# eridgd/WCT-TF

Measured on AMD Instinct MI355X. Metric: stylized frames/sec @512x512, 5-level relu5->1 pipeline, alpha=0.8, higher is better.
Workload: dtype f16

## Files before the change

### wct_tf_amd/csrc/conv.hip

```cpp
#include "common.h"

typedef unsigned int u32x4 __attribute__((ext_vector_type(4)));
constexpr int TW = 16;
constexpr int PITCH = 20;
constexpr int BK = 32;

__device__ __forceinline__ int reflect_idx(int i, int n) {
  if (i < 0) i = -i;
  if (i >= n) i = 2 * n - 2 - i;
  i = i < 0 ? 0 : i;
  return i >= n ? n - 1 : i;
}

template <int MT, int NT, bool POOL, bool OUT32>
__device__ __forceinline__ void conv_epilogue_t(const ConvArgs& p, f32x16 (&acc)[NT][MT], int b, int y0, int x0, int n0,
                                                int wm, int wn, int lane, const unsigned char* bias_lds) {
  typedef _Float16 h2 __attribute__((ext_vector_type(2)));
  constexpr int OOB = (int)0x80000000u;
  const int frag_px = lane & 15;
  const int frag_py = (lane & 31) >> 4;
  const int kgrp = lane >> 5;
  const int Ho = POOL ? (p.H + 1) / 2 : p.H, Wo = POOL ? (p.W + 1) / 2 : p.W;
  const unsigned img_elems = (unsigned)Ho * Wo * p.Cout;
  const __amdgpu_buffer_rsrc_t r16 = __builtin_amdgcn_make_buffer_rsrc(
// ... 73 lines not shown
        __builtin_amdgcn_raw_buffer_store_b128(o, r16, off16 + (nt * 32 + 16 * m) * 2, 0, 0);
      }
    }
  }
  if (stats) umax_merge(p.umax + b * UMAX_SLOTS, (int)blockIdx.x * 4 + (int)(threadIdx.x >> 6), vmax, lane);
}

template <int MT, int NT>
__device__ __forceinline__ void conv_epilogue(const ConvArgs& p, f32x16 (&acc)[NT][MT], int b, int y0, int x0, int n0,
                                              int wm, int wn, int lane, const unsigned char* bias_lds) {
  if (p.pool) conv_epilogue_t<MT, NT, true, false>(p, acc, b, y0, x0, n0, wm, wn, lane, bias_lds);
  else if (p.y32) conv_epilogue_t<MT, NT, false, true>(p, acc, b, y0, x0, n0, wm, wn, lane, bias_lds);
  else conv_epilogue_t<MT, NT, false, false>(p, acc, b, y0, x0, n0, wm, wn, lane, bias_lds);
}

template <int TH, int BN, int WM, int WN, bool FUSE1 = false>
__global__ __launch_bounds__(256, ((TH / 2) / WM) * ((BN / 32) / WN) > 8 ? 1 : 2) void conv3x3_mfma_kernel(ConvArgs p, int tiles_x, int tiles_y, int n_tiles, int strip) {
  constexpr int PH = TH + 2;
  constexpr int MT = (TH / 2) / WM;
  constexpr int NT = (BN / 32) / WN;
  constexpr int PATCH_ITEMS = PH * 18 * 4;
  constexpr int PATCH_PER_THREAD = (PATCH_ITEMS + 255) / 256;
  constexpr int PATCH_BYTES = PH * PITCH * 64;
  constexpr bool DB = MT * NT > 8;
  constexpr int NBUF = DB ? 2 : 1;
  constexpr int DUMP_OFF = PATCH_BYTES;
  constexpr int BUF_STRIDE = PATCH_BYTES + 4096;
  constexpr int BIAS_OFF = NBUF * BUF_STRIDE;
  constexpr int IMG_OFF = BIAS_OFF + BN * 4, IMG_H = TH + 4, IMG_W = 20, IMG_ROW = IMG_W * 3, IMG_ZERO = IMG_OFF + IMG_H * IMG_ROW * 4;
  constexpr int W1_OFF = IMG_ZERO + 64, B1_OFF = W1_OFF + 8192;
  constexpr int STG_OFF = B1_OFF + 256;
  static_assert(!FUSE1 || (BN == 64 && !(((TH / 2) / WM) * ((BN / 32) / WN) > 8)), "FUSE1: 64 output channels, single patch buffer");
  constexpr int PF_TAP = TH <= 16 ? 6 : 9;

  extern __shared__ __attribute__((aligned(16))) unsigned char smem[];
  unsigned char* const patch_lds = smem;

  int bid = blockIdx.x;
  const int ntile = bid % n_tiles;
  bid /= n_tiles;
  const int strips_x = FUSE1 ? (tiles_x + strip - 1) / strip : tiles_x;
  const int tx = FUSE1 ? (bid % strips_x) * strip : bid % strips_x;
  const int ty = bid / strips_x;
  const int b = blockIdx.y;
  int y0 = ty * TH;
  int x0 = tx * TW;
  int strip_i = 0;
  const int n0 = ntile * BN;
  int tid_ = threadIdx.x;

next_tile:
  if (FUSE1) asm volatile("" : "+v"(tid_), "+s"(y0));
  const int tid = tid_;
  const int lane = tid & 63;
  const int wave = tid >> 6;
  const int wm = wave / WN, wn = wave % WN;

  const int Hin = p.upsample ? p.H / 2 : p.H;
  const int Win = p.upsample ? p.W / 2 : p.W;
  const half_t* xb = p.x + (size_t)b * Hin * Win * p.Cin;

  unsigned patch_src[PATCH_PER_THREAD];
  unsigned patch_dst[PATCH_PER_THREAD];
#pragma unroll
  for (int i = 0; i < PATCH_PER_THREAD; ++i) {
    int item = tid + i * 256;
    int valid = item < PATCH_ITEMS;
    int pix = valid ? item >> 2 : 0;
    int chunk = item & 3;
    int py = pix / 18, px = pix - py * 18;
    int iy = reflect_idx(y0 - 1 + py, p.H);
    int ix = reflect_idx(x0 - 1 + px, p.W);
    if (p.upsample) { iy >>= 1; ix >>= 1; }
    patch_src[i] = valid ? ((iy * Win + ix) * p.Cin + chunk * 8) * 2 : 0;
    patch_dst[i] = valid ? ((py * PITCH + px) * 4 + (chunk ^ ((px >> 2) & 3))) * 16 : DUMP_OFF + tid * 16;
  }

  const int frag_px = lane & 15;
  const int frag_py = (lane & 31) >> 4;
  const int kgrp = lane >> 5;

  int rd_base[3][2];
#pragma unroll
  for (int kx = 0; kx < 3; ++kx)
#pragma unroll
    for (int ks = 0; ks < 2; ++ks) {
      const int px = frag_px + kx;
      rd_base[kx][ks] = ((wm * MT * 2 + frag_py) * PITCH + px) * 64 + (((ks * 2 + kgrp) ^ ((px >> 2) & 3)) * 16);
    }

  const int c16 = p.Cin >> 4;
  unsigned wfrag[NT];
#pragma unroll
  for (int nt = 0; nt < NT; ++nt)
    wfrag[nt] = (((n0 >> 5) + wn * NT + nt) * 9 * c16 * 512 + lane * 8) * 2;
  const __amdgpu_buffer_rsrc_t w_rsrc = __builtin_amdgcn_make_buffer_rsrc((void*)p.w, 0, 0x7FFFFFFF, 0x00020000);
  const __amdgpu_buffer_rsrc_t x_rsrc = __builtin_amdgcn_make_buffer_rsrc((void*)xb, 0, 0x7FFFFFFF, 0x00020000);

  f32x16 acc[NT][MT];
  if (tid < BN / 4 && strip_i == 0)
    *reinterpret_cast<f32x4*>(smem + BIAS_OFF + tid * 16) = *reinterpret_cast<const f32x4*>(p.bias + n0 + tid * 4);

  const int n_chunks = p.Cin / BK;
  u32x4 patch_regs[PATCH_PER_THREAD];
  half8 wf[2][NT][2];
  half8 bf[2][MT];

  auto read_group = [&](half8 (&dst)[MT], int ky, int kx, int ks, int buf) {
#pragma unroll
    for (int mt = 0; mt < MT; ++mt)
      dst[mt] = *reinterpret_cast<const half8*>(patch_lds + rd_base[kx][ks] + (mt * 2 + ky) * PITCH * 64 + buf * BUF_STRIDE);
  };
  auto mma_group = [&](half8 (&w)[NT][2], half8 (&bq)[MT], int ks) {
#pragma unroll
    for (int mt = 0; mt < MT; ++mt)
#pragma unroll
      for (int nt = 0; nt < NT; ++nt)
        acc[nt][mt] = __builtin_amdgcn_mfma_f32_32x32x16_f16(w[nt][ks], bq[mt], acc[nt][mt], 0, 0, 0);
  };
  auto load_patch = [&](int chunk) {
#pragma unroll
    for (int i = 0; i < PATCH_PER_THREAD; ++i)
      patch_regs[i] = __builtin_amdgcn_raw_buffer_load_b128(x_rsrc, patch_src[i], chunk * BK * 2, 0);
  };
  auto store_patch = [&](int buf) {
#pragma unroll
// ... 123 lines not shown
  } else {
    load_patch(0);
  }
#pragma unroll
  for (int nt = 0; nt < NT; ++nt)
#pragma unroll
    for (int ks = 0; ks < 2; ++ks)
      wf[0][nt][ks] = __builtin_bit_cast(half8, __builtin_amdgcn_raw_buffer_load_b128(w_rsrc, wfrag[nt] + ks * 1024, 0, 0));
  if (FUSE1) {
    __syncthreads();
    make_patch(0);
  } else {
    store_patch(0);
  }
  __syncthreads();
  read_group(bf[0], 0, 0, 0, 0);

#pragma unroll 1
  for (int pair = 0; pair < n_chunks; pair += 2) {
#pragma unroll
    for (int t = 0; t < 18; ++t) {
      const int tap = t % 9, chunk_i = pair + t / 9;
      const int ky = tap / 3, kx = tap % 3;
      const int ntap = (tap + 1) % 9, nky = ntap / 3, nkx = ntap % 3;
      const bool more = chunk_i + 1 < n_chunks;
      const int buf = DB ? t / 9 : 0;
      {
        const int nchunk = tap == 8 ? (more ? chunk_i + 1 : chunk_i) : chunk_i;
        const int wtap = (ntap * c16 + nchunk * 2) * 1024;
#pragma unroll
        for (int nt = 0; nt < NT; ++nt)
#pragma unroll
          for (int ks = 0; ks < 2; ++ks)
            wf[(t + 1) & 1][nt][ks] =
                __builtin_bit_cast(half8, __builtin_amdgcn_raw_buffer_load_b128(w_rsrc, wfrag[nt] + ks * 1024, wtap, 0));
      }
      if (!FUSE1 && tap == PF_TAP && more) load_patch(chunk_i + 1);
      read_group(bf[1], ky, kx, 1, buf);
      if (DB && tap == 8 && more) store_patch(buf ^ 1);
      __builtin_amdgcn_sched_barrier(0);
      mma_group(wf[t & 1], bf[0], 0);
      __builtin_amdgcn_sched_barrier(0);
      if (tap != 8) {
        read_group(bf[0], nky, nkx, 0, buf);
        __builtin_amdgcn_sched_barrier(0);
        mma_group(wf[t & 1], bf[1], 1);
      } else {
        mma_group(wf[t & 1], bf[1], 1);
        if (more) {
          __syncthreads();
          if (FUSE1) {
            make_patch(chunk_i + 1);
            __syncthreads();
          } else if (!DB) {
            if (PF_TAP > 8) load_patch(chunk_i + 1);
            store_patch(0);
            __syncthreads();
          }
        }
        read_group(bf[0], 0, 0, 0, DB ? buf ^ 1 : 0);
      }
      __builtin_amdgcn_sched_barrier(0);
    }
  }
  const bool more_tiles = FUSE1 && strip_i + 1 < strip && tx + strip_i + 1 < tiles_x;
  if (more_tiles) fetch_img(x0 + TW);
  conv_epilogue<MT, NT>(p, acc, b, y0, x0, n0, wm, wn, lane, smem + BIAS_OFF);
  if (more_tiles) {
    ++strip_i;
    x0 += TW;
    goto next_tile;
  }
}

template <int TH, int BN, int WM, int WN, bool FUSE1 = false>
static int launch_conv_cfg(const ConvArgs& a, hipStream_t s) {
  const int tiles_x = cdiv(a.W, TW), tiles_y = cdiv(a.H, TH);
  const int n_tiles = a.Cout / BN;
  constexpr int PH = TH + 2;
  constexpr int NBUF = ((TH / 2) / WM) * ((BN / 32) / WN) > 8 ? 2 : 1;
  const size_t lds = (size_t)NBUF * (PH * PITCH * 64 + 4096) + BN * sizeof(float)
                     + (FUSE1 ? (size_t)(TH + 4) * 20 * 3 * 4 + 64 + 8192 + 256 + 9 * 1024 : 0);
  const long tiles = (long)tiles_x * tiles_y * a.B;
  const int strip = !FUSE1 ? 1 : tiles >= 8192 ? 4 : tiles >= 4096 ? 2 : 1;
  dim3 grid((FUSE1 ? cdiv(tiles_x, strip) : tiles_x) * tiles_y * n_tiles, a.B);
  if (lds > 64 * 1024) {
    static bool raised[16] = {};
    int dev = 0;
    HIP_TRY(hipGetDevice(&dev));
    if (dev >= 0 && dev < 16 && !raised[dev]) {
      HIP_TRY(hipFuncSetAttribute(reinterpret_cast<const void*>(&conv3x3_mfma_kernel<TH, BN, WM, WN, FUSE1>),
                                  hipFuncAttributeMaxDynamicSharedMemorySize, (int)lds));
      raised[dev] = true;
    }
  }
  hipLaunchKernelGGL((conv3x3_mfma_kernel<TH, BN, WM, WN, FUSE1>), grid, dim3(256), lds, s, a, tiles_x, tiles_y, n_tiles, strip);
  HIP_TRY(hipGetLastError());
  return WCT_OK;
}

int launch_conv3x3(const ConvArgs& a, hipStream_t s) {
  ARG_CHECK(a.Cin % 64 == 0 && a.Cout % 64 == 0 && a.H > 1 && a.W > 1 && a.B > 0);
  ARG_CHECK(!a.upsample || (a.H % 2 == 0 && a.W % 2 == 0));
  ARG_CHECK((size_t)a.H * a.W * a.Cin * 2 < ((size_t)1 << 31));
  ARG_CHECK((size_t)a.H * a.W * a.Cout * (a.y32 ? 4 : 2) < ((size_t)1 << 31));
  ARG_CHECK(!a.usum || (a.y32 && a.umax && a.relu && a.W % 16 == 0));
  ARG_CHECK(!a.pool || (a.relu && !a.y32));
  if (conv3x3_wino_takes(a)) return launch_conv3x3_wino(a, s);
  if (a.img1) {
    ARG_CHECK(a.Cin == 64 && a.Cout == 64 && !a.upsample && a.w1frag && a.bias1);
    return launch_conv_cfg<32, 64, 4, 1, true>(a, s);
  }
  const long px16 = (long)cdiv(a.W, TW) * cdiv(a.H, 16) * a.B;
  const long px32 = (long)cdiv(a.W, TW) * cdiv(a.H, 32) * a.B;
  if (a.Cout % 128 == 0 && px16 * (a.Cout / 128) >= 512) return launch_conv_cfg<16, 128, 2, 2>(a, s);
  if (px32 * (a.Cout / 64) >= 512) return launch_conv_cfg<32, 64, 4, 1>(a, s);
  if (a.Cout % 128 == 0 && px16 * (a.Cout / 128) >= 256) return launch_conv_cfg<16, 128, 2, 2>(a, s);
  if (px16 * (a.Cout / 64) >= 256) return launch_conv_cfg<16, 64, 4, 1>(a, s);
  return launch_conv_cfg<8, 64, 2, 2>(a, s);
}

__global__ __launch_bounds__(256) void conv_first_kernel(ConvFirstArgs p, int strips_x) {
  constexpr int CF_TILES = 4, PATCH_N = 18 * 18 * 3, PER = (PATCH_N + 255) / 256;
  __shared__ float patch[PATCH_N + 4];
  __shared__ __attribute__((aligned(16))) unsigned char tr[4][32 * 256];
  typedef unsigned int u32x4 __attribute__((ext_vector_type(4)));
  const int tid = threadIdx.x, lane = tid & 63, wave = tid >> 6;
  const int sx = blockIdx.x % strips_x, ty = blockIdx.x / strips_x;
  const int b = blockIdx.y;
  const int y0 = ty * 16;
  const float* xb = p.x + (size_t)b * p.H * p.W * 3;
  int e_row[PER], e_px[PER], e_c[PER];
#pragma unroll
  for (int i = 0; i < PER; ++i) {
// ... 286 lines not shown
```

### wct_tf_amd/csrc/conv_wino.hip

```cpp
#include "common.h"

namespace {
typedef unsigned int u32x4 __attribute__((ext_vector_type(4)));
typedef _Float16 h2 __attribute__((ext_vector_type(2)));
constexpr int TW = 16;
constexpr int PITCH = 20;
constexpr int BK = 32;

__device__ __forceinline__ half8 pk_sub(half8 a, half8 b) {
  u32x4 ua = __builtin_bit_cast(u32x4, a), ub = __builtin_bit_cast(u32x4, b), r;
#pragma unroll
  for (int i = 0; i < 4; ++i) {
    unsigned o;
    asm("v_pk_add_f16 %0, %1, %2 neg_lo:[0,1] neg_hi:[0,1]" : "=v"(o) : "v"(ua[i]), "v"(ub[i]));
    r[i] = o;
  }
  return __builtin_bit_cast(half8, r);
}

__device__ __forceinline__ int reflect_idx(int i, int n) {
  if (i < 0) i = -i;
  if (i >= n) i = 2 * n - 2 - i;
  i = i < 0 ? 0 : i;
  return i >= n ? n - 1 : i;
}

template <int TH, int BN, int WM, int WN, bool IL>
__global__ __launch_bounds__(256, TH >= 16 ? 1 : 2)
void conv3x3_wino_kernel(ConvArgs p, int tiles_x, int n_tiles) {
  constexpr int PR = TH / 2;
  constexpr int MT = (PR / 2) / WM;
  constexpr int NT = (BN / 32) / WN;
  constexpr int G = 256 / PR;
  constexpr int SL = (72 + G - 1) / G;
  constexpr int PATCH_BYTES = PR * 4 * PITCH * 64;
  constexpr int DUMP_OFF = 2 * PATCH_BYTES;
  constexpr int PF_TAP = 5;
  static_assert(PR % 2 == 0 && (PR / 2) % WM == 0 && 256 % PR == 0 && WM * WN == 4, "tile shape");

  extern __shared__ __attribute__((aligned(16))) unsigned char smem[];
  const int tid = threadIdx.x, lane = tid & 63, wave = tid >> 6;
  const int wm = wave / WN, wn = wave % WN;
  int bid = blockIdx.x;
  const int ntile = bid % n_tiles;
  bid /= n_tiles;
  const int tx = bid % tiles_x, ty = bid / tiles_x;
  const int b = blockIdx.y;
  const int y0 = ty * TH, x0 = tx * TW, n0 = ntile * BN;

  const int Hin = p.upsample ? p.H / 2 : p.H;
  const int Win = p.upsample ? p.W / 2 : p.W;
  const half_t* xb = p.x + (size_t)b * Hin * Win * p.Cin;
  const __amdgpu_buffer_rsrc_t w_rsrc = __builtin_amdgcn_make_buffer_rsrc((void*)p.w_wino, 0, 0x7FFFFFFF, 0x00020000);
  const __amdgpu_buffer_rsrc_t x_rsrc = __builtin_amdgcn_make_buffer_rsrc((void*)xb, 0, 0x7FFFFFFF, 0x00020000);

  const int lpr = tid / G, ls = tid % G;
  unsigned row_off[4], col_off[SL], dst_off[SL];
  bool slot_ok[SL];
#pragma unroll
  for (int i = 0; i < 4; ++i) {
    int iy = reflect_idx(y0 + 2 * lpr - 1 + i, p.H);
    if (p.upsample) iy >>= 1;
    row_off[i] = (unsigned)(iy * Win) * p.Cin * 2;
  }
#pragma unroll
  for (int j = 0; j < SL; ++j) {
    const int slot = ls + j * G;
    slot_ok[j] = slot < 72;
    const int px = slot_ok[j] ? slot >> 2 : 0, piece = slot & 3;
    int ix = reflect_idx(x0 - 1 + px, p.W);
    if (p.upsample) ix >>= 1;
    col_off[j] = (unsigned)(ix * p.Cin + piece * 8) * 2;
    dst_off[j] = ((lpr * 4 * PITCH + px) * 4 + (piece ^ ((px >> 2) & 3))) * 16;
    if (IL && !slot_ok[j]) dst_off[j] = DUMP_OFF + tid * 16;
  }
  u32x4 raw[SL][4];
  auto load_rows = [&](int chunk) {
#pragma unroll
    for (int j = 0; j < SL; ++j)
#pragma unroll
      for (int i = 0; i < 4; ++i)
        raw[j][i] = __builtin_amdgcn_raw_buffer_load_b128(x_rsrc, row_off[i] + col_off[j], chunk * BK * 2, 0);
  };
  auto park_rows = [&](int buf) {
#pragma unroll
    for (int j = 0; j < SL; ++j) {
      const half8 d0 = __builtin_bit_cast(half8, raw[j][0]), d1 = __builtin_bit_cast(half8, raw[j][1]);
      const half8 d2 = __builtin_bit_cast(half8, raw[j][2]), d3 = __builtin_bit_cast(half8, raw[j][3]);
      const half8 t0 = pk_sub(d0, d2), t1 = d1 + d2, t2 = pk_sub(d2, d1), t3 = pk_sub(d1, d3);
      if (slot_ok[j]) {
        unsigned char* d = smem + buf * PATCH_BYTES + dst_off[j];
        *reinterpret_cast<half8*>(d) = t0;
        *reinterpret_cast<half8*>(d + PITCH * 64) = t1;
        *reinterpret_cast<half8*>(d + 2 * PITCH * 64) = t2;
        *reinterpret_cast<half8*>(d + 3 * PITCH * 64) = t3;
      }
    }
  };

  const int frag_px = lane & 15, frag_pr = (lane & 31) >> 4, kgrp = lane >> 5;
  int rd_base[3][2];
#pragma unroll
  for (int kx = 0; kx < 3; ++kx)
#pragma unroll
    for (int ks = 0; ks < 2; ++ks) {
      const int px = frag_px + kx;
      rd_base[kx][ks] = (((wm * MT * 2 + frag_pr) * 4) * PITCH + px) * 64 + (((ks * 2 + kgrp) ^ ((px >> 2) & 3)) * 16);
    }
  const int c16 = p.Cin >> 4;
  unsigned wfrag[NT];
#pragma unroll
  for (int nt = 0; nt < NT; ++nt) wfrag[nt] = (((n0 >> 5) + wn * NT + nt) * 12 * c16 * 512 + lane * 8) * 2;

  f32x16 acc[4][NT][MT];
#pragma unroll
  for (int nt = 0; nt < NT; ++nt) {
    f32x4 bv[4];
#pragma unroll
    for (int rq = 0; rq < 4; ++rq) bv[rq] = *reinterpret_cast<const f32x4*>(p.bias + n0 + (wn * NT + nt) * 32 + 8 * rq + 4 * kgrp);
#pragma unroll
    for (int f = 0; f < 4; ++f)
#pragma unroll
      for (int mt = 0; mt < MT; ++mt)
#pragma unroll
        for (int r = 0; r < 16; ++r) acc[f][nt][mt][r] = f == 1 ? bv[r >> 2][r & 3] : 0.f;
  }

  const int n_chunks = p.Cin / BK;
  half8 wf[3][NT][2];
  half8 bf[IL ? 3 : 2][2][MT];
  auto load_w = [&](half8 (&dst)[NT][2], int tap12, int chunk) {
    const int soff = (tap12 * c16 + chunk * 2) * 1024;
#pragma unroll
    for (int nt = 0; nt < NT; ++nt)
#pragma unroll
      for (int ks = 0; ks < 2; ++ks)
// ... 2 lines not shown
  auto read_b = [&](half8 (&dst)[2][MT], int f, int kx, int buf) {
#pragma unroll
    for (int ks = 0; ks < 2; ++ks)
#pragma unroll
      for (int mt = 0; mt < MT; ++mt)
        dst[ks][mt] = *reinterpret_cast<const half8*>(smem + buf * PATCH_BYTES + rd_base[kx][ks] + (mt * 8 + f) * PITCH * 64);
  };

  if constexpr (IL) {
    constexpr int NM = 2 * MT * NT;
    constexpr int NR = 2 * NT + 2 * MT;
#ifndef WINO_LT0
#define WINO_LT0 1
#define WINO_PT0 6
#endif
    constexpr int LT0 = WINO_LT0, PT0 = WINO_PT0;
    static_assert(LT0 + SL <= PT0 && PT0 + SL <= 10, "staging schedule");
#ifndef WINO_WRING
#define WINO_WRING 4
#endif
#ifndef WINO_ABL
#define WINO_ABL 0
#endif
#ifndef WINO_RAW_AUX
#define WINO_RAW_AUX 0
#endif
    constexpr int ABL = WINO_ABL;
    constexpr int WR = WINO_WRING, WA = WR - 1;
    static_assert(24 % WR == 0, "ring");
    half8 wq[WR][NT][2];
    half8 tq[4];
    load_rows(0);
#pragma unroll
    for (int i = 0; i < WA; ++i) load_w(wq[i], i, 0);
#pragma unroll
    for (int j = 0; j < SL; ++j) {
      const half8 d0 = __builtin_bit_cast(half8, raw[j][0]), d1 = __builtin_bit_cast(half8, raw[j][1]);
      const half8 d2 = __builtin_bit_cast(half8, raw[j][2]), d3 = __builtin_bit_cast(half8, raw[j][3]);
      unsigned char* d = smem + dst_off[j];
      *reinterpret_cast<half8*>(d) = pk_sub(d0, d2);
      *reinterpret_cast<half8*>(d + PITCH * 64) = d1 + d2;
      *reinterpret_cast<half8*>(d + 2 * PITCH * 64) = pk_sub(d2, d1);
      *reinterpret_cast<half8*>(d + 3 * PITCH * 64) = pk_sub(d1, d3);
    }
    asm volatile("s_waitcnt lgkmcnt(0)\n\ts_barrier" ::: "memory");
    read_b(bf[0], 0, 0, 0);
    read_b(bf[1], 0, 1, 0);
#pragma unroll 1
    for (int pair = 0; pair < n_chunks; pair += 2) {
#pragma unroll
      for (int t = 0; t < 24; ++t) {
        const int tt = t % 12, chunk_i = pair + t / 12, buf = t / 12;
        const int f = tt / 3, kx = tt % 3;
        const int chunk_n = chunk_i + 1 < n_chunks ? chunk_i + 1 : chunk_i;
        const int t3 = (tt + WA) % 12, c3 = tt + WA >= 12 ? chunk_n : chunk_i;
        const int t1 = (tt + 2) % 12, buf1 = tt >= 10 ? buf ^ 1 : buf;
        const int soff3 = (t3 * c16 + c3 * 2) * 1024;
#pragma unroll
        for (int j = 0; j < NM; ++j) {
          const int ks = j / (MT * NT), mt = (j / NT) % MT, nt = j % NT;
          if (!(ABL & 4)) acc[f][nt][mt] = __builtin_amdgcn_mfma_f32_32x32x16_f16(wq[t % WR][nt][ks], bf[t % 3][ks][mt], acc[f][nt][mt], 0, 0, 0);
          else asm volatile("" :: "v"(wq[t % WR][nt][ks]), "v"(bf[t % 3][ks][mt]));
#pragma unroll
          for (int k = j * NR / NM; k < (j + 1) * NR / NM; ++k) {
            if (k < 2 * NT) {
              if (!(ABL & 1)) wq[(t + WA) % WR][k / 2][k % 2] =
                  __builtin_bit_cast(half8, __builtin_amdgcn_raw_buffer_load_b128(w_rsrc, wfrag[k / 2] + (k % 2) * 1024, soff3, 0));
            } else {
              const int kk = k - 2 * NT, ks1 = kk / MT, mt1 = kk % MT;
              if (!(ABL & 8)) bf[(t + 2) % 3][ks1][mt1] = *reinterpret_cast<const half8*>(smem + buf1 * PATCH_BYTES + rd_base[t1 % 3][ks1] + (mt1 * 8 + t1 / 3) * PITCH * 64);
            }
          }
          if (tt >= LT0 && tt < LT0 + SL) {
            const int sl = tt - LT0;
            if (j < 4 && !(ABL & 2)) raw[sl][j] = __builtin_amdgcn_raw_buffer_load_b128(x_rsrc, (ABL & 64) ? (lane & 3) * 16 + j * 64 + sl * 256 : row_off[j] + col_off[sl], (ABL & 32) ? 0 : chunk_n * BK * 2, WINO_RAW_AUX);
          }
          if (tt >= PT0 && tt < PT0 + SL && !(ABL & 16)) {
            const int sl = tt - PT0;
            {
#pragma unroll
              for (int it = j * 8 / NM; it < (j + 1) * 8 / NM; ++it) {
                const int fq = it >> 1;
                if ((it & 1) == 0) {
                  const half8 da = __builtin_bit_cast(half8, raw[sl][fq == 0 ? 0 : fq == 1 ? 1 : fq == 2 ? 2 : 1]);
                  const half8 db = __builtin_bit_cast(half8, raw[sl][fq == 0 ? 2 : fq == 1 ? 2 : fq == 2 ? 1 : 3]);
                  tq[fq] = fq == 1 ? da + db : pk_sub(da, db);
                } else {
                  *reinterpret_cast<half8*>(smem + (buf ^ 1) * PATCH_BYTES * (slot_ok[sl] ? 1 : 0) + dst_off[sl] + fq * PITCH * 64) = tq[fq];
                }
              }
            }
          }
          __builtin_amdgcn_sched_barrier(0);
        }
        if (tt == 9) asm volatile("s_waitcnt lgkmcnt(0)\n\ts_barrier" ::: "memory");
      }
    }
  } else {
  load_rows(0);
  load_w(wf[0], 0, 0);
  load_w(wf[1], 1, 0);
  park_rows(0);
  asm volatile("s_waitcnt lgkmcnt(0)\n\ts_barrier" ::: "memory");
  read_b(bf[0], 0, 0, 0);

#pragma unroll 1
  for (int pair = 0; pair < n_chunks; pair += 2) {
#pragma unroll
    for (int t = 0; t < 24; ++t) {
      const int tt = t % 12, chunk_i = pair + t / 12, buf = t / 12;
      const int f = tt / 3, kx = tt % 3;
      const bool more = chunk_i + 1 < n_chunks;
      {
        const int t2 = (tt + 2) % 12;
        const int c2 = tt + 2 >= 12 ? (more ? chunk_i + 1 : chunk_i) : chunk_i;
        load_w(wf[(t + 2) % 3], t2, c2);
      }
      if (tt == PF_TAP && more) load_rows(chunk_i + 1);
      if (tt != 11) read_b(bf[(t + 1) & 1], (tt + 1) / 3, (tt + 1) % 3, buf);
      else if (more) read_b(bf[(t + 1) & 1], 0, 0, buf ^ 1);
      __builtin_amdgcn_sched_barrier(0);
#pragma unroll
      for (int ks = 0; ks < 2; ++ks)
#pragma unroll
        for (int mt = 0; mt < MT; ++mt)
#pragma unroll
          for (int nt = 0; nt < NT; ++nt)
            acc[f][nt][mt] = __builtin_amdgcn_mfma_f32_32x32x16_f16(wf[t % 3][nt][ks], bf[t & 1][ks][mt], acc[f][nt][mt], 0, 0, 0);
      __builtin_amdgcn_sched_barrier(0);
      if (tt == 10 && more) {
        park_rows(buf ^ 1);
        asm volatile("s_waitcnt lgkmcnt(0)\n\ts_barrier" ::: "memory");
      }
    }
  }

  }
  constexpr int OOB = (int)0x80000000u;
  const int Ho = p.pool ? (p.H + 1) / 2 : p.H, Wo = p.pool ? (p.W + 1) / 2 : p.W;
  const unsigned img_elems = (unsigned)Ho * Wo * p.Cout;
  const __amdgpu_buffer_rsrc_t r16 = __builtin_amdgcn_make_buffer_rsrc((void*)(p.y16 + (size_t)b * img_elems), 0, img_elems * 2, 0x00020000);
  const float lo1 = p.relu ? 0.f : -__builtin_inff();
  const h2 lo2 = {(half_t)lo1, (half_t)lo1};
  const h2 zero2 = {(half_t)0.f, (half_t)0.f};
  const int ox = x0 + frag_px;
// ... 7 lines not shown
      off[0] = in0 && (frag_px & 1) == 0 ? (((oy >> 1) * Wo + (ox >> 1)) * p.Cout + chan + 8 * kgrp) * 2 : OOB;
      off[1] = OOB;
    } else {
      off[0] = in0 ? ((oy * p.W + ox) * p.Cout + chan + 8 * kgrp) * 2 : OOB;
      off[1] = in1 ? (((oy + 1) * p.W + ox) * p.Cout + chan + 8 * kgrp) * 2 : OOB;
    }
#pragma unroll
    for (int nt = 0; nt < NT; ++nt) {
      unsigned pk[2][4][2];
#pragma unroll
      for (int rq = 0; rq < 4; ++rq) {
        f32x4 e, o;
#pragma unroll
        for (int j = 0; j < 4; ++j) {
          const int r = rq * 4 + j;
          const float m0 = acc[0][nt][mt][r], m1 = acc[1][nt][mt][r], m2 = acc[2][nt][mt][r], m3 = acc[3][nt][mt][r];
          e[j] = (m0 + m1) + m2;
          o[j] = (m1 - m2) - m3;
        }
        h2 e0 = {(half_t)e[0], (half_t)e[1]}, e1 = {(half_t)e[2], (half_t)e[3]};
        h2 o0 = {(half_t)o[0], (half_t)o[1]}, o1 = {(half_t)o[2], (half_t)o[3]};
        e0 = __builtin_elementwise_max(e0, lo2); e1 = __builtin_elementwise_max(e1, lo2);
        o0 = __builtin_elementwise_max(o0, lo2); o1 = __builtin_elementwise_max(o1, lo2);
        if (p.pool) {
          h2 q[2] = {__builtin_elementwise_max(in0 ? e0 : zero2, in1 ? o0 : zero2), __builtin_elementwise_max(in0 ? e1 : zero2, in1 ? o1 : zero2)};
#pragma unroll
          for (int d = 0; d < 2; ++d) {
            const unsigned tq = __builtin_bit_cast(unsigned, q[d]);
            const h2 nb = __builtin_bit_cast(h2, __builtin_amdgcn_update_dpp(0, (int)tq, 0xB1, 0xF, 0xF, true));
            q[d] = __builtin_elementwise_max(q[d], nb);
          }
          e0 = q[0]; e1 = q[1];
        }
// ... 2 lines not shown
      }
#pragma unroll
      for (int par = 0; par < 2; ++par) {
#pragma unroll
        for (int m = 0; m < 2; ++m) {
          auto sx = __builtin_amdgcn_permlane32_swap(pk[par][2 * m][0], pk[par][2 * m + 1][0], false, false);
          auto sy = __builtin_amdgcn_permlane32_swap(pk[par][2 * m][1], pk[par][2 * m + 1][1], false, false);
          u32x4 ov = {sx[0], sy[0], sx[1], sy[1]};
          __builtin_amdgcn_raw_buffer_store_b128(ov, r16, off[par] + (nt * 32 + 16 * m) * 2, 0, 0);
        }
      }
    }
  }
}

template <int TH, int BN, int WM, int WN, bool IL = false>
int launch_wino_cfg(const ConvArgs& a, hipStream_t s) {
  const int tiles_x = cdiv(a.W, TW), tiles_y = cdiv(a.H, TH), n_tiles = a.Cout / BN;
  const size_t lds = 2 * (size_t)(TH / 2) * 4 * PITCH * 64 + (IL ? 8192 : 0);
  HIP_TRY(hipFuncSetAttribute(reinterpret_cast<const void*>(&conv3x3_wino_kernel<TH, BN, WM, WN, IL>),
                              hipFuncAttributeMaxDynamicSharedMemorySize, (int)lds));
  hipLaunchKernelGGL((conv3x3_wino_kernel<TH, BN, WM, WN, IL>), dim3(tiles_x * tiles_y * n_tiles, a.B), dim3(256), lds, s, a, tiles_x, n_tiles);
  HIP_TRY(hipGetLastError());
  return WCT_OK;
}
}

bool conv3x3_wino_takes(const ConvArgs& a) {
  return a.w_wino != nullptr && a.y16 != nullptr && a.y32 == nullptr && a.usum == nullptr && a.img1 == nullptr &&
         a.Cin % 64 == 0 && a.Cout % 64 == 0 && (!a.pool || a.relu);
}

int launch_conv3x3_wino(const ConvArgs& a, hipStream_t s) {
  ARG_CHECK(conv3x3_wino_takes(a) && a.H > 1 && a.W > 1 && a.B > 0);
  ARG_CHECK(!a.upsample || (a.H % 2 == 0 && a.W % 2 == 0));
  ARG_CHECK((size_t)a.H * a.W * a.Cin * 2 < ((size_t)1 << 31));
  ARG_CHECK((size_t)a.H * a.W * a.Cout * 2 < ((size_t)1 << 31));
  const long px16 = (long)cdiv(a.W, TW) * cdiv(a.H, 16) * a.B;
  const long px8 = (long)cdiv(a.W, TW) * cdiv(a.H, 8) * a.B;
  if (a.Cout % 128 == 0 && px16 * (a.Cout / 128) >= 256) return launch_wino_cfg<16, 128, 1, 4, true>(a, s);
  if (a.Cout % 128 == 0 && px8 * (a.Cout / 128) >= 256) return launch_wino_cfg<8, 128, 1, 4>(a, s);
  return launch_wino_cfg<8, 64, 2, 2>(a, s);
}
```

Baseline: 662.6.

## Specialize 3x3 convs with fused nearest upsample to exploit duplicated input rows

Adds an UP template path to both the direct MFMA conv and the Winograd conv, used when the conv input is a 2x nearest-upsampled activation. The direct kernel stages only the half-resolution patch with 8 channel chunks per pixel and reads it with remapped, swizzled LDS addressing. It also refreshes the patch only every other chunk, which cuts global loads and barriers. The Winograd kernel uses the fact that adjacent upsampled rows are equal: it drops one of the four row-transform planes (3 filters and 9 taps instead of 4 and 12) and shortens the MFMA loop and the epilogue. The cost is more complex indexing, extra template instantiations and a larger register and LDS footprint, with correctness depending on the reflection and duplication mapping being right at tile edges.

```diff
diff --git a/wct_tf_amd/csrc/conv.hip b/wct_tf_amd/csrc/conv.hip
--- a/wct_tf_amd/csrc/conv.hip
+++ b/wct_tf_amd/csrc/conv.hip
@@ -111,14 +111,18 @@
   else conv_epilogue_t<MT, NT, false, false>(p, acc, b, y0, x0, n0, wm, wn, lane, bias_lds);
 }
 
-template <int TH, int BN, int WM, int WN, bool FUSE1 = false>
+template <int TH, int BN, int WM, int WN, bool FUSE1 = false, bool UP = false>
 __global__ __launch_bounds__(256, ((TH / 2) / WM) * ((BN / 32) / WN) > 8 ? 1 : 2) void conv3x3_mfma_kernel(ConvArgs p, int tiles_x, int tiles_y, int n_tiles, int strip) {
-  constexpr int PH = TH + 2;
+  constexpr int PH = UP ? TH / 2 + 2 : TH + 2;
   constexpr int MT = (TH / 2) / WM;
   constexpr int NT = (BN / 32) / WN;
-  constexpr int PATCH_ITEMS = PH * 18 * 4;
+  constexpr int PW = UP ? 10 : 18;
+  constexpr int PP = UP ? 11 : PITCH;
+  constexpr int PC = UP ? 8 : 4;
+  constexpr int PXB = PC * 16;
+  constexpr int PATCH_ITEMS = PH * PW * PC;
   constexpr int PATCH_PER_THREAD = (PATCH_ITEMS + 255) / 256;
-  constexpr int PATCH_BYTES = PH * PITCH * 64;
+  constexpr int PATCH_BYTES = PH * PP * PXB;
   constexpr bool DB = MT * NT > 8;
   constexpr int NBUF = DB ? 2 : 1;
   constexpr int DUMP_OFF = PATCH_BYTES;
@@ -127,6 +131,7 @@
   constexpr int IMG_OFF = BIAS_OFF + BN * 4, IMG_H = TH + 4, IMG_W = 20, IMG_ROW = IMG_W * 3, IMG_ZERO = IMG_OFF + IMG_H * IMG_ROW * 4;
   constexpr int W1_OFF = IMG_ZERO + 64, B1_OFF = W1_OFF + 8192;
   constexpr int STG_OFF = B1_OFF + 256;
+  static_assert(!UP || (!FUSE1 && !DB), "UP: activations in, single patch buffer");
   static_assert(!FUSE1 || (BN == 64 && !(((TH / 2) / WM) * ((BN / 32) / WN) > 8)), "FUSE1: 64 output channels, single patch buffer");
   constexpr int PF_TAP = TH <= 16 ? 6 : 9;
 
@@ -153,8 +158,8 @@
   const int wave = tid >> 6;
   const int wm = wave / WN, wn = wave % WN;
 
-  const int Hin = p.upsample ? p.H / 2 : p.H;
-  const int Win = p.upsample ? p.W / 2 : p.W;
+  const int Hin = UP ? p.H / 2 : p.H;
+  const int Win = UP ? p.W / 2 : p.W;
   const half_t* xb = p.x + (size_t)b * Hin * Win * p.Cin;
 
   unsigned patch_src[PATCH_PER_THREAD];
@@ -163,14 +168,15 @@
   for (int i = 0; i < PATCH_PER_THREAD; ++i) {
     int item = tid + i * 256;
     int valid = item < PATCH_ITEMS;
-    int pix = valid ? item >> 2 : 0;
-    int chunk = item & 3;
-    int py = pix / 18, px = pix - py * 18;
-    int iy = reflect_idx(y0 - 1 + py, p.H);
-    int ix = reflect_idx(x0 - 1 + px, p.W);
-    if (p.upsample) { iy >>= 1; ix >>= 1; }
+    int pix = valid ? item / PC : 0;
+    int chunk = item % PC;
+    int py = pix / PW, px = pix - py * PW;
+    int iy = reflect_idx(UP ? (py == 0 ? y0 - 1 : y0 + 2 * (py - 1)) : y0 - 1 + py, p.H);
+    int ix = reflect_idx(UP ? (px == 0 ? x0 - 1 : x0 + 2 * (px - 1)) : x0 - 1 + px, p.W);
+    if (UP) { iy >>= 1; ix >>= 1; }
+    const int sw = UP ? (px >> 1) ^ ((px & 1) << 2) : (px >> 2) & 3;
     patch_src[i] = valid ? ((iy * Win + ix) * p.Cin + chunk * 8) * 2 : 0;
-    patch_dst[i] = valid ? ((py * PITCH + px) * 4 + (chunk ^ ((px >> 2) & 3))) * 16 : DUMP_OFF + tid * 16;
+    patch_dst[i] = valid ? ((py * PP + px) * PC + (chunk ^ sw)) * 16 : DUMP_OFF + tid * 16;
   }
 
   const int frag_px = lane & 15;
@@ -182,8 +188,13 @@
   for (int kx = 0; kx < 3; ++kx)
 #pragma unroll
     for (int ks = 0; ks < 2; ++ks) {
-      const int px = frag_px + kx;
-      rd_base[kx][ks] = ((wm * MT * 2 + frag_py) * PITCH + px) * 64 + (((ks * 2 + kgrp) ^ ((px >> 2) & 3)) * 16);
+      if (UP) {
+        const int c = (frag_px + kx + 1) >> 1, row = wm * MT + (ks ? 1 : frag_py);
+        rd_base[kx][ks] = (row * PP + c) * PXB + ((((c >> 1) ^ ((c & 1) << 2)) ^ kgrp) * 16);
+      } else {
+        const int px = frag_px + kx;
+        rd_base[kx][ks] = ((wm * MT * 2 + frag_py) * PITCH + px) * 64 + (((ks * 2 + kgrp) ^ ((px >> 2) & 3)) * 16);
+      }
     }
 
   const int c16 = p.Cin >> 4;
@@ -203,10 +214,17 @@
   half8 wf[2][NT][2];
   half8 bf[2][MT];
 
-  auto read_group = [&](half8 (&dst)[MT], int ky, int kx, int ks, int buf) {
-#pragma unroll
-    for (int mt = 0; mt < MT; ++mt)
-      dst[mt] = *reinterpret_cast<const half8*>(patch_lds + rd_base[kx][ks] + (mt * 2 + ky) * PITCH * 64 + buf * BUF_STRIDE);
+  auto read_group = [&](half8 (&dst)[MT], int ky, int kx, int ks, int buf, int hf) {
+    if (UP) {
+      const int a = rd_base[kx][ky == 1] ^ ((hf * 4 + ks * 2) * 16);
+#pragma unroll
+      for (int mt = 0; mt < MT; ++mt)
+        dst[mt] = *reinterpret_cast<const half8*>(patch_lds + a + (mt + (ky == 2)) * PP * PXB);
+    } else {
+#pragma unroll
+      for (int mt = 0; mt < MT; ++mt)
+        dst[mt] = *reinterpret_cast<const half8*>(patch_lds + rd_base[kx][ks] + (mt * 2 + ky) * PITCH * 64 + buf * BUF_STRIDE);
+    }
   };
   auto mma_group = [&](half8 (&w)[NT][2], half8 (&bq)[MT], int ks) {
 #pragma unroll
@@ -360,10 +378,14 @@
     store_patch(0);
   }
   __syncthreads();
-  read_group(bf[0], 0, 0, 0, 0);
+  read_group(bf[0], 0, 0, 0, 0, 0);
 
 #pragma unroll 1
   for (int pair = 0; pair < n_chunks; pair += 2) {
+    if (UP) {
+#pragma unroll
+      for (int i = 0; i < 6; ++i) asm volatile("" : "+v"(rd_base[i / 2][i % 2]));
+    }
 #pragma unroll
     for (int t = 0; t < 18; ++t) {
       const int tap = t % 9, chunk_i = pair + t / 9;
@@ -371,6 +393,7 @@
       const int ntap = (tap + 1) % 9, nky = ntap / 3, nkx = ntap % 3;
       const bool more = chunk_i + 1 < n_chunks;
       const int buf = DB ? t / 9 : 0;
+      const int hf = UP ? t / 9 : 0;
       {
         const int nchunk = tap == 8 ? (more ? chunk_i + 1 : chunk_i) : chunk_i;
         const int wtap = (ntap * c16 + nchunk * 2) * 1024;
@@ -381,19 +404,19 @@
             wf[(t + 1) & 1][nt][ks] =
                 __builtin_bit_cast(half8, __builtin_amdgcn_raw_buffer_load_b128(w_rsrc, wfrag[nt] + ks * 1024, wtap, 0));
       }
-      if (!FUSE1 && tap == PF_TAP && more) load_patch(chunk_i + 1);
-      read_group(bf[1], ky, kx, 1, buf);
+      if (!FUSE1 && tap == PF_TAP && more && (!UP || hf)) load_patch(chunk_i + 1);
+      read_group(bf[1], ky, kx, 1, buf, hf);
       if (DB && tap == 8 && more) store_patch(buf ^ 1);
       __builtin_amdgcn_sched_barrier(0);
       mma_group(wf[t & 1], bf[0], 0);
       __builtin_amdgcn_sched_barrier(0);
       if (tap != 8) {
-        read_group(bf[0], nky, nkx, 0, buf);
+        read_group(bf[0], nky, nkx, 0, buf, hf);
         __builtin_amdgcn_sched_barrier(0);
         mma_group(wf[t & 1], bf[1], 1);
       } else {
         mma_group(wf[t & 1], bf[1], 1);
-        if (more) {
+        if (more && (!UP || hf)) {
           __syncthreads();
           if (FUSE1) {
             make_patch(chunk_i + 1);
@@ -404,7 +427,7 @@
             __syncthreads();
           }
         }
-        read_group(bf[0], 0, 0, 0, DB ? buf ^ 1 : 0);
+        read_group(bf[0], 0, 0, 0, DB ? buf ^ 1 : 0, hf ^ (UP ? 1 : 0));
       }
       __builtin_amdgcn_sched_barrier(0);
     }
@@ -419,13 +442,13 @@
   }
 }
 
-template <int TH, int BN, int WM, int WN, bool FUSE1 = false>
+template <int TH, int BN, int WM, int WN, bool FUSE1 = false, bool UP = false>
 static int launch_conv_cfg(const ConvArgs& a, hipStream_t s) {
   const int tiles_x = cdiv(a.W, TW), tiles_y = cdiv(a.H, TH);
   const int n_tiles = a.Cout / BN;
-  constexpr int PH = TH + 2;
+  constexpr int PH = UP ? TH / 2 + 2 : TH + 2;
   constexpr int NBUF = ((TH / 2) / WM) * ((BN / 32) / WN) > 8 ? 2 : 1;
-  const size_t lds = (size_t)NBUF * (PH * PITCH * 64 + 4096) + BN * sizeof(float)
+  const size_t lds = (size_t)NBUF * ((UP ? PH * 11 * 128 : PH * PITCH * 64) + 4096) + BN * sizeof(float)
                      + (FUSE1 ? (size_t)(TH + 4) * 20 * 3 * 4 + 64 + 8192 + 256 + 9 * 1024 : 0);
   const long tiles = (long)tiles_x * tiles_y * a.B;
   const int strip = !FUSE1 ? 1 : tiles >= 8192 ? 4 : tiles >= 4096 ? 2 : 1;
@@ -435,12 +458,12 @@
     int dev = 0;
     HIP_TRY(hipGetDevice(&dev));
     if (dev >= 0 && dev < 16 && !raised[dev]) {
-      HIP_TRY(hipFuncSetAttribute(reinterpret_cast<const void*>(&conv3x3_mfma_kernel<TH, BN, WM, WN, FUSE1>),
+      HIP_TRY(hipFuncSetAttribute(reinterpret_cast<const void*>(&conv3x3_mfma_kernel<TH, BN, WM, WN, FUSE1, UP>),
                                   hipFuncAttributeMaxDynamicSharedMemorySize, (int)lds));
       raised[dev] = true;
     }
   }
-  hipLaunchKernelGGL((conv3x3_mfma_kernel<TH, BN, WM, WN, FUSE1>), grid, dim3(256), lds, s, a, tiles_x, tiles_y, n_tiles, strip);
+  hipLaunchKernelGGL((conv3x3_mfma_kernel<TH, BN, WM, WN, FUSE1, UP>), grid, dim3(256), lds, s, a, tiles_x, tiles_y, n_tiles, strip);
   HIP_TRY(hipGetLastError());
   return WCT_OK;
 }
@@ -459,11 +482,13 @@
   }
   const long px16 = (long)cdiv(a.W, TW) * cdiv(a.H, 16) * a.B;
   const long px32 = (long)cdiv(a.W, TW) * cdiv(a.H, 32) * a.B;
-  if (a.Cout % 128 == 0 && px16 * (a.Cout / 128) >= 512) return launch_conv_cfg<16, 128, 2, 2>(a, s);
-  if (px32 * (a.Cout / 64) >= 512) return launch_conv_cfg<32, 64, 4, 1>(a, s);
-  if (a.Cout % 128 == 0 && px16 * (a.Cout / 128) >= 256) return launch_conv_cfg<16, 128, 2, 2>(a, s);
-  if (px16 * (a.Cout / 64) >= 256) return launch_conv_cfg<16, 64, 4, 1>(a, s);
-  return launch_conv_cfg<8, 64, 2, 2>(a, s);
+#define CONV_CFG(...) (a.upsample ? launch_conv_cfg<__VA_ARGS__, false, true>(a, s) : launch_conv_cfg<__VA_ARGS__>(a, s))
+  if (a.Cout % 128 == 0 && px16 * (a.Cout / 128) >= 512) return CONV_CFG(16, 128, 2, 2);
+  if (px32 * (a.Cout / 64) >= 512) return CONV_CFG(32, 64, 4, 1);
+  if (a.Cout % 128 == 0 && px16 * (a.Cout / 128) >= 256) return CONV_CFG(16, 128, 2, 2);
+  if (px16 * (a.Cout / 64) >= 256) return CONV_CFG(16, 64, 4, 1);
+  return CONV_CFG(8, 64, 2, 2);
+#undef CONV_CFG
 }
 
 __global__ __launch_bounds__(256) void conv_first_kernel(ConvFirstArgs p, int strips_x) {
diff --git a/wct_tf_amd/csrc/conv_wino.hip b/wct_tf_amd/csrc/conv_wino.hip
--- a/wct_tf_amd/csrc/conv_wino.hip
+++ b/wct_tf_amd/csrc/conv_wino.hip
@@ -25,17 +25,23 @@
   return i >= n ? n - 1 : i;
 }
 
-template <int TH, int BN, int WM, int WN, bool IL>
+template <int TH, int BN, int WM, int WN, bool IL, bool UP>
 __global__ __launch_bounds__(256, TH >= 16 ? 1 : 2)
 void conv3x3_wino_kernel(ConvArgs p, int tiles_x, int n_tiles) {
   constexpr int PR = TH / 2;
   constexpr int MT = (PR / 2) / WM;
   constexpr int NT = (BN / 32) / WN;
   constexpr int G = 256 / PR;
-  constexpr int SL = (72 + G - 1) / G;
+  constexpr int NF = UP ? 3 : 4;
+  constexpr int NTAP = NF * 3;
+  constexpr int NRAW = UP ? 3 : 4;
+  constexpr int NS = UP ? 40 : 72;
+  constexpr int SL = (NS + G - 1) / G;
   constexpr int PATCH_BYTES = PR * 4 * PITCH * 64;
   constexpr int DUMP_OFF = 2 * PATCH_BYTES;
-  constexpr int PF_TAP = 5;
+  constexpr int PF_TAP = NTAP - 7;
+  auto FQ = [](int i) { return UP && i == 2 ? 3 : i; };
+  auto TAP12 = [](int t) { return UP && t >= 6 ? t + 3 : t; };
   static_assert(PR % 2 == 0 && (PR / 2) % WM == 0 && 256 % PR == 0 && WM * WN == 4, "tile shape");
 
   extern __shared__ __attribute__((aligned(16))) unsigned char smem[];
@@ -48,43 +54,68 @@
   const int b = blockIdx.y;
   const int y0 = ty * TH, x0 = tx * TW, n0 = ntile * BN;
 
-  const int Hin = p.upsample ? p.H / 2 : p.H;
-  const int Win = p.upsample ? p.W / 2 : p.W;
+  const bool ups = UP || p.upsample;
+  const int Hin = ups ? p.H / 2 : p.H;
+  const int Win = ups ? p.W / 2 : p.W;
   const half_t* xb = p.x + (size_t)b * Hin * Win * p.Cin;
   const __amdgpu_buffer_rsrc_t w_rsrc = __builtin_amdgcn_make_buffer_rsrc((void*)p.w_wino, 0, 0x7FFFFFFF, 0x00020000);
   const __amdgpu_buffer_rsrc_t x_rsrc = __builtin_amdgcn_make_buffer_rsrc((void*)xb, 0, 0x7FFFFFFF, 0x00020000);
 
   const int lpr = tid / G, ls = tid % G;
-  unsigned row_off[4], col_off[SL], dst_off[SL];
-  bool slot_ok[SL];
-#pragma unroll
-  for (int i = 0; i < 4; ++i) {
-    int iy = reflect_idx(y0 + 2 * lpr - 1 + i, p.H);
-    if (p.upsample) iy >>= 1;
+  unsigned row_off[NRAW], col_off[SL], dst_off[SL], dst_off2[UP ? SL : 1];
+  bool slot_ok[SL], slot_two[UP ? SL : 1];
+#pragma unroll
+  for (int i = 0; i < NRAW; ++i) {
+    int iy = reflect_idx(y0 + 2 * lpr - 1 + FQ(i), p.H);
+    if (ups) iy >>= 1;
     row_off[i] = (unsigned)(iy * Win) * p.Cin * 2;
   }
 #pragma unroll
   for (int j = 0; j < SL; ++j) {
     const int slot = ls + j * G;
-    slot_ok[j] = slot < 72;
-    const int px = slot_ok[j] ? slot >> 2 : 0, piece = slot & 3;
-    int ix = reflect_idx(x0 - 1 + px, p.W);
-    if (p.upsample) ix >>= 1;
+    slot_ok[j] = slot < NS;
+    const int col = slot_ok[j] ? slot >> 2 : 0, piece = slot & 3;
+    const int px1 = UP ? (col == 0 ? 0 : 2 * col - 1) : col;
+    const int px = UP ? (col & 1 ? 2 * col - 1 : 2 * col) : col;
+    int ix = reflect_idx(x0 - 1 + px1, p.W);
+    if (ups) ix >>= 1;
     col_off[j] = (unsigned)(ix * p.Cin + piece * 8) * 2;
     dst_off[j] = ((lpr * 4 * PITCH + px) * 4 + (piece ^ ((px >> 2) & 3))) * 16;
     if (IL && !slot_ok[j]) dst_off[j] = DUMP_OFF + tid * 16;
-  }
-  u32x4 raw[SL][4];
+    if (UP) {
+      slot_two[j] = slot_ok[j] && col >= 1 && col <= 8;
+      const int px2 = col & 1 ? 2 * col : 2 * col - 1;
+      dst_off2[j] = ((lpr * 4 * PITCH + px2) * 4 + (piece ^ ((px2 >> 2) & 3))) * 16;
+      if (IL && !slot_two[j]) dst_off2[j] = DUMP_OFF + tid * 16;
+    }
+  }
+  u32x4 raw[SL][NRAW];
   auto load_rows = [&](int chunk) {
 #pragma unroll
     for (int j = 0; j < SL; ++j)
 #pragma unroll
-      for (int i = 0; i < 4; ++i)
+      for (int i = 0; i < NRAW; ++i)
         raw[j][i] = __builtin_amdgcn_raw_buffer_load_b128(x_rsrc, row_off[i] + col_off[j], chunk * BK * 2, 0);
   };
   auto park_rows = [&](int buf) {
 #pragma unroll
     for (int j = 0; j < SL; ++j) {
+      if constexpr (UP) {
+        const half8 d0 = __builtin_bit_cast(half8, raw[j][0]), d1 = __builtin_bit_cast(half8, raw[j][1]), d3 = __builtin_bit_cast(half8, raw[j][2]);
+        const half8 t0 = pk_sub(d0, d1), t1 = d1 + d1, t3 = pk_sub(d1, d3);
+        if (slot_ok[j]) {
+          unsigned char* d = smem + buf * PATCH_BYTES + dst_off[j];
+          *reinterpret_cast<half8*>(d) = t0;
+          *reinterpret_cast<half8*>(d + PITCH * 64) = t1;
+          *reinterpret_cast<half8*>(d + 3 * PITCH * 64) = t3;
+        }
+        if (slot_two[j]) {
+          unsigned char* d = smem + buf * PATCH_BYTES + dst_off2[j];
+          *reinterpret_cast<half8*>(d) = t0;
+          *reinterpret_cast<half8*>(d + PITCH * 64) = t1;
+          *reinterpret_cast<half8*>(d + 3 * PITCH * 64) = t3;
+        }
+      } else {
       const half8 d0 = __builtin_bit_cast(half8, raw[j][0]), d1 = __builtin_bit_cast(half8, raw[j][1]);
       const half8 d2 = __builtin_bit_cast(half8, raw[j][2]), d3 = __builtin_bit_cast(half8, raw[j][3]);
       const half8 t0 = pk_sub(d0, d2), t1 = d1 + d2, t2 = pk_sub(d2, d1), t3 = pk_sub(d1, d3);
@@ -95,6 +126,7 @@
         *reinterpret_cast<half8*>(d + 2 * PITCH * 64) = t2;
         *reinterpret_cast<half8*>(d + 3 * PITCH * 64) = t3;
       }
+      }
     }
   };
 
@@ -112,14 +144,14 @@
 #pragma unroll
   for (int nt = 0; nt < NT; ++nt) wfrag[nt] = (((n0 >> 5) + wn * NT + nt) * 12 * c16 * 512 + lane * 8) * 2;
 
-  f32x16 acc[4][NT][MT];
+  f32x16 acc[NF][NT][MT];
 #pragma unroll
   for (int nt = 0; nt < NT; ++nt) {
     f32x4 bv[4];
 #pragma unroll
     for (int rq = 0; rq < 4; ++rq) bv[rq] = *reinterpret_cast<const f32x4*>(p.bias + n0 + (wn * NT + nt) * 32 + 8 * rq + 4 * kgrp);
 #pragma unroll
-    for (int f = 0; f < 4; ++f)
+    for (int f = 0; f < NF; ++f)
 #pragma unroll
       for (int mt = 0; mt < MT; ++mt)
 #pragma unroll
@@ -152,8 +184,8 @@
 #define WINO_LT0 1
 #define WINO_PT0 6
 #endif
-    constexpr int LT0 = WINO_LT0, PT0 = WINO_PT0;
-    static_assert(LT0 + SL <= PT0 && PT0 + SL <= 10, "staging schedule");
+    constexpr int LT0 = UP ? 0 : WINO_LT0, PT0 = UP ? 5 : WINO_PT0;
+    static_assert(LT0 + SL <= PT0 && PT0 + SL <= NTAP - 2, "staging schedule");
 #ifndef WINO_WRING
 #define WINO_WRING 4
 #endif
@@ -164,15 +196,27 @@
 #define WINO_RAW_AUX 0
 #endif
     constexpr int ABL = WINO_ABL;
-    constexpr int WR = WINO_WRING, WA = WR - 1;
-    static_assert(24 % WR == 0, "ring");
+    constexpr int WR = UP ? 6 : WINO_WRING, WA = UP ? 3 : WR - 1;
+    static_assert((2 * NTAP) % WR == 0 && WA < WR, "ring");
     half8 wq[WR][NT][2];
     half8 tq[4];
     load_rows(0);
 #pragma unroll
-    for (int i = 0; i < WA; ++i) load_w(wq[i], i, 0);
+    for (int i = 0; i < WA; ++i) load_w(wq[i], TAP12(i), 0);
 #pragma unroll
     for (int j = 0; j < SL; ++j) {
+      if constexpr (UP) {
+        const half8 d0 = __builtin_bit_cast(half8, raw[j][0]), d1 = __builtin_bit_cast(half8, raw[j][1]), d3 = __builtin_bit_cast(half8, raw[j][2]);
+        const half8 t0 = pk_sub(d0, d1), t1 = d1 + d1, t3 = pk_sub(d1, d3);
+        unsigned char* d = smem + dst_off[j];
+        unsigned char* e = smem + dst_off2[j];
+        *reinterpret_cast<half8*>(d) = t0;
+        *reinterpret_cast<half8*>(e) = t0;
+        *reinterpret_cast<half8*>(d + PITCH * 64) = t1;
+        *reinterpret_cast<half8*>(e + PITCH * 64) = t1;
+        *reinterpret_cast<half8*>(d + 3 * PITCH * 64) = t3;
+        *reinterpret_cast<half8*>(e + 3 * PITCH * 64) = t3;
+      } else {
       const half8 d0 = __builtin_bit_cast(half8, raw[j][0]), d1 = __builtin_bit_cast(half8, raw[j][1]);
       const half8 d2 = __builtin_bit_cast(half8, raw[j][2]), d3 = __builtin_bit_cast(half8, raw[j][3]);
       unsigned char* d = smem + dst_off[j];
@@ -180,6 +224,7 @@
       *reinterpret_cast<half8*>(d + PITCH * 64) = d1 + d2;
       *reinterpret_cast<half8*>(d + 2 * PITCH * 64) = pk_sub(d2, d1);
       *reinterpret_cast<half8*>(d + 3 * PITCH * 64) = pk_sub(d1, d3);
+      }
     }
     asm volatile("s_waitcnt lgkmcnt(0)\n\ts_barrier" ::: "memory");
     read_b(bf[0], 0, 0, 0);
@@ -187,13 +232,13 @@
 #pragma unroll 1
     for (int pair = 0; pair < n_chunks; pair += 2) {
 #pragma unroll
-      for (int t = 0; t < 24; ++t) {
-        const int tt = t % 12, chunk_i = pair + t / 12, buf = t / 12;
+      for (int t = 0; t < 2 * NTAP; ++t) {
+        const int tt = t % NTAP, chunk_i = pair + t / NTAP, buf = t / NTAP;
         const int f = tt / 3, kx = tt % 3;
         const int chunk_n = chunk_i + 1 < n_chunks ? chunk_i + 1 : chunk_i;
-        const int t3 = (tt + WA) % 12, c3 = tt + WA >= 12 ? chunk_n : chunk_i;
-        const int t1 = (tt + 2) % 12, buf1 = tt >= 10 ? buf ^ 1 : buf;
-        const int soff3 = (t3 * c16 + c3 * 2) * 1024;
+        const int t3 = (tt + WA) % NTAP, c3 = tt + WA >= NTAP ? chunk_n : chunk_i;
+        const int t1 = (tt + 2) % NTAP, buf1 = tt >= NTAP - 2 ? buf ^ 1 : buf;
+        const int soff3 = (TAP12(t3) * c16 + c3 * 2) * 1024;
 #pragma unroll
         for (int j = 0; j < NM; ++j) {
           const int ks = j / (MT * NT), mt = (j / NT) % MT, nt = j % NT;
@@ -206,16 +251,30 @@
                   __builtin_bit_cast(half8, __builtin_amdgcn_raw_buffer_load_b128(w_rsrc, wfrag[k / 2] + (k % 2) * 1024, soff3, 0));
             } else {
               const int kk = k - 2 * NT, ks1 = kk / MT, mt1 = kk % MT;
-              if (!(ABL & 8)) bf[(t + 2) % 3][ks1][mt1] = *reinterpret_cast<const half8*>(smem + buf1 * PATCH_BYTES + rd_base[t1 % 3][ks1] + (mt1 * 8 + t1 / 3) * PITCH * 64);
+              if (!(ABL & 8)) bf[(t + 2) % 3][ks1][mt1] = *reinterpret_cast<const half8*>(smem + buf1 * PATCH_BYTES + rd_base[t1 % 3][ks1] + (mt1 * 8 + FQ(t1 / 3)) * PITCH * 64);
             }
           }
           if (tt >= LT0 && tt < LT0 + SL) {
             const int sl = tt - LT0;
-            if (j < 4 && !(ABL & 2)) raw[sl][j] = __builtin_amdgcn_raw_buffer_load_b128(x_rsrc, (ABL & 64) ? (lane & 3) * 16 + j * 64 + sl * 256 : row_off[j] + col_off[sl], (ABL & 32) ? 0 : chunk_n * BK * 2, WINO_RAW_AUX);
+            if (j < NRAW && !(ABL & 2)) raw[sl][j] = __builtin_amdgcn_raw_buffer_load_b128(x_rsrc, (ABL & 64) ? (lane & 3) * 16 + j * 64 + sl * 256 : row_off[j] + col_off[sl], (ABL & 32) ? 0 : chunk_n * BK * 2, WINO_RAW_AUX);
           }
           if (tt >= PT0 && tt < PT0 + SL && !(ABL & 16)) {
             const int sl = tt - PT0;
-            {
+            if constexpr (UP) {
+#pragma unroll
+              for (int it = j * 9 / NM; it < (j + 1) * 9 / NM; ++it) {
+                const int fi = it / 3, r = it % 3;
+                if (r == 0) {
+                  const half8 da = __builtin_bit_cast(half8, raw[sl][fi == 0 ? 0 : 1]);
+                  const half8 db = __builtin_bit_cast(half8, raw[sl][fi == 2 ? 2 : 1]);
+                  tq[fi] = fi == 1 ? da + db : pk_sub(da, db);
+                } else if (r == 1) {
+                  *reinterpret_cast<half8*>(smem + (buf ^ 1) * PATCH_BYTES * (slot_ok[sl] ? 1 : 0) + dst_off[sl] + FQ(fi) * PITCH * 64) = tq[fi];
+                } else {
+                  *reinterpret_cast<half8*>(smem + (buf ^ 1) * PATCH_BYTES * (slot_two[sl] ? 1 : 0) + dst_off2[sl] + FQ(fi) * PITCH * 64) = tq[fi];
+                }
+              }
+            } else {
 #pragma unroll
               for (int it = j * 8 / NM; it < (j + 1) * 8 / NM; ++it) {
                 const int fq = it >> 1;
@@ -231,13 +290,13 @@
           }
           __builtin_amdgcn_sched_barrier(0);
         }
-        if (tt == 9) asm volatile("s_waitcnt lgkmcnt(0)\n\ts_barrier" ::: "memory");
+        if (tt == NTAP - 3) asm volatile("s_waitcnt lgkmcnt(0)\n\ts_barrier" ::: "memory");
       }
     }
   } else {
   load_rows(0);
-  load_w(wf[0], 0, 0);
-  load_w(wf[1], 1, 0);
+  load_w(wf[0], TAP12(0), 0);
+  load_w(wf[1], TAP12(1), 0);
   park_rows(0);
   asm volatile("s_waitcnt lgkmcnt(0)\n\ts_barrier" ::: "memory");
   read_b(bf[0], 0, 0, 0);
@@ -245,17 +304,17 @@
 #pragma unroll 1
   for (int pair = 0; pair < n_chunks; pair += 2) {
 #pragma unroll
-    for (int t = 0; t < 24; ++t) {
-      const int tt = t % 12, chunk_i = pair + t / 12, buf = t / 12;
+    for (int t = 0; t < 2 * NTAP; ++t) {
+      const int tt = t % NTAP, chunk_i = pair + t / NTAP, buf = t / NTAP;
       const int f = tt / 3, kx = tt % 3;
       const bool more = chunk_i + 1 < n_chunks;
       {
-        const int t2 = (tt + 2) % 12;
-        const int c2 = tt + 2 >= 12 ? (more ? chunk_i + 1 : chunk_i) : chunk_i;
-        load_w(wf[(t + 2) % 3], t2, c2);
+        const int t2 = (tt + 2) % NTAP;
+        const int c2 = tt + 2 >= NTAP ? (more ? chunk_i + 1 : chunk_i) : chunk_i;
+        load_w(wf[(t + 2) % 3], TAP12(t2), c2);
       }
       if (tt == PF_TAP && more) load_rows(chunk_i + 1);
-      if (tt != 11) read_b(bf[(t + 1) & 1], (tt + 1) / 3, (tt + 1) % 3, buf);
+      if (tt != NTAP - 1) read_b(bf[(t + 1) & 1], FQ((tt + 1) / 3), (tt + 1) % 3, buf);
       else if (more) read_b(bf[(t + 1) & 1], 0, 0, buf ^ 1);
       __builtin_amdgcn_sched_barrier(0);
 #pragma unroll
@@ -266,7 +325,7 @@
           for (int nt = 0; nt < NT; ++nt)
             acc[f][nt][mt] = __builtin_amdgcn_mfma_f32_32x32x16_f16(wf[t % 3][nt][ks], bf[t & 1][ks][mt], acc[f][nt][mt], 0, 0, 0);
       __builtin_amdgcn_sched_barrier(0);
-      if (tt == 10 && more) {
+      if (tt == NTAP - 2 && more) {
         park_rows(buf ^ 1);
         asm volatile("s_waitcnt lgkmcnt(0)\n\ts_barrier" ::: "memory");
       }
@@ -304,9 +363,15 @@
 #pragma unroll
         for (int j = 0; j < 4; ++j) {
           const int r = rq * 4 + j;
+          if constexpr (UP) {
+            const float m0 = acc[0][nt][mt][r], m1 = acc[1][nt][mt][r], m3 = acc[2][nt][mt][r];
+            e[j] = m0 + m1;
+            o[j] = m1 - m3;
+          } else {
           const float m0 = acc[0][nt][mt][r], m1 = acc[1][nt][mt][r], m2 = acc[2][nt][mt][r], m3 = acc[3][nt][mt][r];
           e[j] = (m0 + m1) + m2;
           o[j] = (m1 - m2) - m3;
+          }
         }
         h2 e0 = {(half_t)e[0], (half_t)e[1]}, e1 = {(half_t)e[2], (half_t)e[3]};
         h2 o0 = {(half_t)o[0], (half_t)o[1]}, o1 = {(half_t)o[2], (half_t)o[3]};
@@ -339,13 +404,13 @@
   }
 }
 
-template <int TH, int BN, int WM, int WN, bool IL = false>
+template <int TH, int BN, int WM, int WN, bool IL, bool UP>
 int launch_wino_cfg(const ConvArgs& a, hipStream_t s) {
   const int tiles_x = cdiv(a.W, TW), tiles_y = cdiv(a.H, TH), n_tiles = a.Cout / BN;
   const size_t lds = 2 * (size_t)(TH / 2) * 4 * PITCH * 64 + (IL ? 8192 : 0);
-  HIP_TRY(hipFuncSetAttribute(reinterpret_cast<const void*>(&conv3x3_wino_kernel<TH, BN, WM, WN, IL>),
+  HIP_TRY(hipFuncSetAttribute(reinterpret_cast<const void*>(&conv3x3_wino_kernel<TH, BN, WM, WN, IL, UP>),
                               hipFuncAttributeMaxDynamicSharedMemorySize, (int)lds));
-  hipLaunchKernelGGL((conv3x3_wino_kernel<TH, BN, WM, WN, IL>), dim3(tiles_x * tiles_y * n_tiles, a.B), dim3(256), lds, s, a, tiles_x, n_tiles);
+  hipLaunchKernelGGL((conv3x3_wino_kernel<TH, BN, WM, WN, IL, UP>), dim3(tiles_x * tiles_y * n_tiles, a.B), dim3(256), lds, s, a, tiles_x, n_tiles);
   HIP_TRY(hipGetLastError());
   return WCT_OK;
 }
@@ -363,7 +428,9 @@
   ARG_CHECK((size_t)a.H * a.W * a.Cout * 2 < ((size_t)1 << 31));
   const long px16 = (long)cdiv(a.W, TW) * cdiv(a.H, 16) * a.B;
   const long px8 = (long)cdiv(a.W, TW) * cdiv(a.H, 8) * a.B;
-  if (a.Cout % 128 == 0 && px16 * (a.Cout / 128) >= 256) return launch_wino_cfg<16, 128, 1, 4, true>(a, s);
-  if (a.Cout % 128 == 0 && px8 * (a.Cout / 128) >= 256) return launch_wino_cfg<8, 128, 1, 4>(a, s);
-  return launch_wino_cfg<8, 64, 2, 2>(a, s);
-}
+#define WINO_CFG(...) (a.upsample ? launch_wino_cfg<__VA_ARGS__, true>(a, s) : launch_wino_cfg<__VA_ARGS__, false>(a, s))
+  if (a.Cout % 128 == 0 && px16 * (a.Cout / 128) >= 256) return WINO_CFG(16, 128, 1, 4, true);
+  if (a.Cout % 128 == 0 && px8 * (a.Cout / 128) >= 256) return WINO_CFG(8, 128, 1, 4, false);
+  return WINO_CFG(8, 64, 2, 2, false);
+#undef WINO_CFG
+}
```

Result: no change. 668.0, median of 6 (+0.8%).
